# neoyinyao/Recommender

Measured on AMD Instinct MI355X. Metric: examples/sec fwd+bwd, Criteo-DLRM 26×40M×128 batch 65536, 1/2/4/8 GPU, higher is better.
Workload: dtype fp32; 1 GPU; dlrm_criteo_26x40000000x128; global_batch=65536, per_gpu_batch=65536, rows=40000000, dim=128, slots=26, optimizer=sgd, parallelism=single, prefetch=False

## Files before the change

### recommender_amd/csrc/interaction.hip

```cpp
#include <map>
#include <mutex>
#include <tuple>
#include <type_traits>

#include "common.hpp"

namespace rs {

int32_t fold_two_level(const float* part, int nchunks, int N, float* part2, float* out,
                       hipStream_t st);

typedef float floatx4 __attribute__((ext_vector_type(4)));
typedef float floatx16 __attribute__((ext_vector_type(16)));

struct InterMode {
  int self_interaction;
  int skip_gather;
};

__device__ __forceinline__ bool keep_pair(int i, int j, int self_i) {
  return self_i ? (i >= j) : (i < j);
}
__device__ __forceinline__ int compact_index(int i, int j, int F, int self_i) {
  return self_i ? (i * (i + 1) / 2 + j) : (i * F - i * (i + 1) / 2 + (j - i - 1));
// ... 434 lines not shown
      const float gsc = gscale[bb];
#pragma unroll
      for (int j = 0; j < GREG; ++j) gnx[j] = gsc * pv[j];
    } else {
      gfloat* grow = (gfloat*)(gout + bb * gstride);
#pragma unroll
      for (int j = 0; j < GREG; ++j) gnx[j] = grow[min(ln + 64 * j, glast)];
    }
  };
  const float* cur = row_of(first, raw_id(first));
  int64_t id_next = raw_id(first + 1);
#pragma unroll
  for (int s = 0; s < KS; ++s) load_rows(cur, s);
  load_g(first, lane);
  float* gs = gsm[wave];
  if (lane == 0) gs[ZS] = 0.f;
  for (int64_t b = first; b < last; ++b) {
    int lanev;
    asm volatile("v_mbcnt_lo_u32_b32 %0, -1, 0\n\tv_mbcnt_hi_u32_b32 %0, -1, %0" : "=v"(lanev));
    const int r = lanev & 31, h = lanev >> 5;
#pragma unroll
    for (int j = 0; j < GREG; ++j) gs[lane + 64 * j] = gnx[j];
    const float* nxt = row_of(b + 1, id_next);
    id_next = raw_id(b + 2);
    __builtin_amdgcn_s_waitcnt(0xc07f);
    __builtin_amdgcn_wave_barrier();
    float sa[KS];
#pragma unroll
    for (int s = 0; s < KS; ++s) {
      const int k = 2 * s + h;
      const bool in = r < F && k < F;
      const bool p1 = in && keep_pair(r, k, SELF);
      const bool p2 = in && keep_pair(k, r, SELF);
      const int j1 = p1 ? (SKIP ? r * F + k : compact_index(r, k, F, SELF)) : ZS;
      const int j2 = p2 ? (SKIP ? k * F + r : compact_index(k, r, F, SELF)) : ZS;
      sa[s] = gs[j1] + gs[j2];
    }
    floatx16 acc[NTILE];
#pragma unroll
    for (int c = 0; c < NTILE; ++c)
#pragma unroll
      for (int e = 0; e < 16; ++e) acc[c][e] = 0.f;
#pragma unroll
    for (int s = 0; s < KS; ++s) {
#pragma unroll
      for (int c = 0; c < NTILE; ++c)
        acc[c] = __builtin_amdgcn_mfma_f32_32x32x2f32(sa[s], xv[s][c], acc[c], 0, 0, 0);
    }
    __builtin_amdgcn_sched_barrier(0);
#pragma unroll
    for (int s = 0; s < KS; ++s) load_rows(nxt, s);
    __builtin_amdgcn_sched_barrier(0);
    float dpass[NTILE];
#pragma unroll
    for (int c = 0; c < NTILE; ++c) dpass[c] = gs[nz + NTILE * r + c];
    load_g(b + 1, lanev);
#pragma unroll
    for (int reg = 0; reg < 16; ++reg) {
      const int i = (reg & 3) + 8 * (reg >> 2) + 4 * h;
      if (i < F) {
        float v[NTILE];
#pragma unroll
        for (int c = 0; c < NTILE; ++c) v[c] = acc[c][reg] + (i == S ? dpass[c] : 0.f);
        float* dst = (i < S ? gemb + (b * S + i) * (int64_t)D : gdense + b * D) + NTILE * r;
        *reinterpret_cast<float4*>(dst) = make_float4(v[0], v[1], v[2], v[3]);
      }
    }
  }
  if (__any(oob) && lane == 0) flag_oob(src.err_flag);
}

constexpr int kDxLdx = 136;
constexpr int kDxRows = 28;
constexpr int kDxZt = 32 * 33;

template <bool ID64>
__global__ __launch_bounds__(256) void dlrm_fwd_dx_pipe(GatherSrc src, int64_t batch, int F,
                                                        float* __restrict__ out,
                                                        int64_t out_stride, FwdHead hd, int epw) {
  constexpr int D = 128, NT = 8;
  __shared__ __attribute__((aligned(16))) float lds[4][kDxRows * kDxLdx + kDxZt];
  const int wave = threadIdx.x >> 6, lane = threadIdx.x & 63;
  const int64_t first = ((int64_t)blockIdx.x * 4 + wave) * epw;
  if (first >= batch) return;
  const int64_t last = first + epw < batch ? first + epw : batch;
  const int r = lane & 15, g = lane >> 4;
  const int r32 = lane & 31, h = lane >> 5;
  const int S = src.n_slots;
  const int nzc = F * (F - 1) / 2;
  float* X = lds[wave];
  float(*z)[33] = reinterpret_cast<float(*)[33]>(lds[wave] + kDxRows * kDxLdx);
  float qz[8], qd[2], sa[2][8], qdn[4];
#pragma unroll
  for (int t = 0; t < 8; ++t) qz[t] = lane + 64 * t < nzc ? hd.q[lane + 64 * t] : 0.f;
#pragma unroll
  for (int t = 0; t < 2; ++t) qd[t] = hd.q[nzc + lane + 64 * t];
  const float cc = hd.c[0];
#pragma unroll
  for (int ib = 0; ib < 2; ++ib)
#pragma unroll
    for (int kk = 0; kk < 8; ++kk) {
      const int m = 16 * ib + r, k = 4 * kk + g;
      const bool in = m < F && k < F && m != k;
      const float v = hd.q[in ? compact_index(m < k ? m : k, m < k ? k : m, F, 0) : 0];
      sa[ib][kk] = in ? v : 0.f;
    }
#pragma unroll
  for (int c = 0; c < 4; ++c) qdn[c] = hd.q[nzc + 4 * r32 + c];
  int zoff[8];
#pragma unroll
  for (int t = 0; t < 8; ++t) {
    const int o = lane + 64 * t;
    int i = 0, j = 0;
    if (o < nzc) compact_pair(o, F, false, i, j);
    zoff[t] = o < nzc ? i * 33 + j : -1;
  }
  int64_t lo = 0, n_ok = src.n_rows;
  if (lane < S && src.slot_offsets) {
    lo = src.slot_offsets[lane];
    n_ok = src.slot_offsets[lane + 1] - lo;
  }
  bool oob = false;
  auto raw_id = [&](int64_t b) -> int64_t {
    const int64_t bb = b < last ? b : first;
    const int ln = lane < S ? lane : S - 1;
    const int64_t v = ID64 ? static_cast<const int64_t*>(src.ids)[bb * S + ln]
                           : static_cast<int64_t>(static_cast<const int32_t*>(src.ids)[bb * S + ln]);
    return lane < S ? v : 0;
  };
  auto row_of = [&](int64_t b, int64_t id) -> const float* {
    const bool live = b < last;
    const bool id_ok = id >= 0 && id < n_ok;
    if (lane < S && !id_ok && live) oob = true;
    if (lane < S) return id_ok ? src.table + (lo + id) * D : kZeroRow;
    return (lane == S && live) ? src.dense + (b < last ? b : first) * D : kZeroRow;
  };
  floatx4 a0[NT], a1[NT];
  float dnv[2];
  auto gather = [&](const float* mine, int64_t b) {
    const float* p0 = shfl_ptr(mine, r);
    const float* p1 = shfl_ptr(mine, 16 + r);
#pragma unroll
    for (int t = 0; t < NT; ++t) {
      a0[t] = *(gfloatx4*)(p0 + 4 * g + 16 * t);
      a1[t] = *(gfloatx4*)(p1 + 4 * g + 16 * t);
    }
    const int64_t bb = b < last ? b : first;
#pragma unroll
    for (int t = 0; t < 2; ++t) dnv[t] = *(gfloat*)(src.dense + bb * D + lane + 64 * t);
  };
  gather(row_of(first, raw_id(first)), first);
  int64_t id_next = raw_id(first + 1);
  for (int64_t b = first; b < last; ++b) {
    int lanev;
    asm volatile("v_mbcnt_lo_u32_b32 %0, -1, 0\n\tv_mbcnt_hi_u32_b32 %0, -1, %0" : "=v"(lanev));
    const int r = lanev & 15, g = (lanev >> 4) & 3;
    const int r32 = lanev & 31, h = (lanev >> 5) & 1;
    const float* nxt = row_of(b + 1, id_next);
    id_next = raw_id(b + 2);
    floatx4 c00 = {0.f, 0.f, 0.f, 0.f}, c01 = c00, c11 = c00;
#pragma unroll
    for (int t = 0; t < NT; ++t) {
#pragma unroll
      for (int c = 0; c < 4; ++c) {
        c00 = __builtin_amdgcn_mfma_f32_16x16x4f32(a0[t][c], a0[t][c], c00, 0, 0, 0);
        c01 = __builtin_amdgcn_mfma_f32_16x16x4f32(a0[t][c], a1[t][c], c01, 0, 0, 0);
        c11 = __builtin_amdgcn_mfma_f32_16x16x4f32(a1[t][c], a1[t][c], c11, 0, 0, 0);
      }
    }
#pragma unroll
    for (int t = 0; t < NT; ++t) {
      *reinterpret_cast<floatx4*>(&X[r * kDxLdx + 16 * t + 4 * g]) = a0[t];
      if (16 + r < kDxRows) *reinterpret_cast<floatx4*>(&X[(16 + r) * kDxLdx + 16 * t + 4 * g]) = a1[t];
    }
    float dn_cur[2] = {dnv[0], dnv[1]};
    __builtin_amdgcn_sched_barrier(0);
    gather(nxt, b + 1);
    __builtin_amdgcn_sched_barrier(0);
#pragma unroll
    for (int reg = 0; reg < 4; ++reg) {
      const int i = 4 * g + reg;
      z[i][r] = c00[reg];
      z[i][16 + r] = c01[reg];
      z[16 + r][i] = c01[reg];
      z[16 + i][16 + r] = c11[reg];
    }
    __builtin_amdgcn_wave_barrier();
    float* orow = out + b * out_stride;
    float hacc = 0.f;
    const int pad = nzc + D;
#pragma unroll
    for (int t = 0; t < 8; ++t) {
      const int o = lanev + 64 * t;
      const bool in = zoff[t] >= 0;
      const float v = in ? (&z[0][0])[zoff[t]] : 0.f;
      orow[in ? o : pad] = v;
      hacc += v * qz[t];
    }
    float* od = orow + nzc;
#pragma unroll
    for (int t = 0; t < 2; ++t) {
      const int d = lanev + 64 * t;
      od[d] = dn_cur[t];
      hacc += dn_cur[t] * qd[t];
    }
#pragma unroll
    for (int off = 32; off > 0; off >>= 1) hacc += __shfl_xor(hacc, off);
    {
      const float v = hacc + cc;
      hd.y[b] = hd.act == 2 ? 1.f / (1.f + expf(-v)) : (hd.act == 1 ? fmaxf(v, 0.f) : v);
    }
    {
      const int o = pad + lanev;
      orow[o < out_stride ? o : pad] = 0.f;
    }
#pragma unroll
    for (int t = 0; t < NT; ++t) {
      constexpr int KK = kDxRows / 4;
      float bv[KK];
#pragma unroll
      for (int kk = 0; kk < KK; ++kk) bv[kk] = X[(4 * kk + g) * kDxLdx + 16 * t + r];
      floatx4 d0 = {0.f, 0.f, 0.f, 0.f}, d1 = d0;
#pragma unroll
      for (int kk = 0; kk < KK; ++kk) {
        d0 = __builtin_amdgcn_mfma_f32_16x16x4f32(sa[0][kk], bv[kk], d0, 0, 0, 0);
        d1 = __builtin_amdgcn_mfma_f32_16x16x4f32(sa[1][kk], bv[kk], d1, 0, 0, 0);
      }
#pragma unroll
      for (int reg = 0; reg < 4; ++reg) {
        const int i0 = 4 * g + reg, i1 = 16 + 4 * g + reg;
        X[i0 * kDxLdx + 16 * t + r] = d0[reg];
        if (i1 < kDxRows) X[i1 * kDxLdx + 16 * t + r] = d1[reg];
      }
    }
    __builtin_amdgcn_wave_barrier();
    float* de = hd.dxu_emb + b * S * (int64_t)D;
#pragma unroll
    for (int s2 = 0; s2 < kDxRows / 2; ++s2) {
      const int i = 2 * s2 + h < S ? 2 * s2 + h : S;
      floatx4 v = *reinterpret_cast<const floatx4*>(&X[i * kDxLdx + 4 * r32]);
      const bool emb = i < S;
#pragma unroll
      for (int c = 0; c < 4; ++c) v[c] = emb ? v[c] : v[c] + qdn[c];
      float* dst = emb ? de + i * D : hd.dxu_dense + b * D;
      *reinterpret_cast<floatx4*>(dst + 4 * r32) = v;
    }
    __builtin_amdgcn_wave_barrier();
  }
  if (__any(oob) && lane == 0) flag_oob(src.err_flag);
}

typedef __bf16 bf16x8 __attribute__((ext_vector_type(8)));

typedef __bf16 bf16x2 __attribute__((ext_vector_type(2)));
typedef float floatx2 __attribute__((ext_vector_type(2)));
__device__ __forceinline__ void split3(const floatx4& lo, const floatx4& hi, bf16x8& h, bf16x8& m,
                                       bf16x8& l) {
#pragma unroll
  for (int j = 0; j < 4; ++j) {
    const floatx2 x = j < 2 ? floatx2{lo[2 * j], lo[2 * j + 1]} : floatx2{hi[2 * j - 4], hi[2 * j - 3]};
    const bf16x2 hp = __builtin_convertvector(x, bf16x2);
    const floatx2 r1 = x - __builtin_convertvector(hp, floatx2);
    const bf16x2 mp = __builtin_convertvector(r1, bf16x2);
    const bf16x2 lp = __builtin_convertvector(r1 - __builtin_convertvector(mp, floatx2), bf16x2);
    h[2 * j] = hp[0];
    h[2 * j + 1] = hp[1];
    m[2 * j] = mp[0];
    m[2 * j + 1] = mp[1];
    l[2 * j] = lp[0];
    l[2 * j + 1] = lp[1];
  }
}

__device__ __forceinline__ floatx4 mfma6(const bf16x8& ah, const bf16x8& am, const bf16x8& al,
                                         const bf16x8& bh, const bf16x8& bm, const bf16x8& bl,
                                         floatx4 c) {
  c = __builtin_amdgcn_mfma_f32_16x16x32_bf16(am, bm, c, 0, 0, 0);
  c = __builtin_amdgcn_mfma_f32_16x16x32_bf16(ah, bl, c, 0, 0, 0);
  c = __builtin_amdgcn_mfma_f32_16x16x32_bf16(al, bh, c, 0, 0, 0);
  c = __builtin_amdgcn_mfma_f32_16x16x32_bf16(ah, bm, c, 0, 0, 0);
  c = __builtin_amdgcn_mfma_f32_16x16x32_bf16(am, bh, c, 0, 0, 0);
  return __builtin_amdgcn_mfma_f32_16x16x32_bf16(ah, bh, c, 0, 0, 0);
}

constexpr int kTrainAtop = 512;
constexpr int kTrainNI = 13;
template <int D>
constexpr int train_m() { return kTrainAtop + 2 + kTrainNI * D + D; }
constexpr int kTrainM = train_m<128>();

struct TrainArgs {
  const float* q;
  const float* c;
  const float* label;
  const float* xin;
  float eps;
  float gscale;
  float* y;
  float* grad_emb;
  float* part;
};

typedef short shortx4 __attribute__((ext_vector_type(4)));
typedef short shortx8 __attribute__((ext_vector_type(8)));
typedef __attribute__((address_space(3))) shortx4 lds_shortx4;

__device__ __forceinline__ floatx4 mfma6_xs(const bf16x8& xh, const bf16x8& xm, const bf16x8& xl,
                                            const bf16x8& sh, const bf16x8& sm, const bf16x8& sl,
                                            floatx4 c) {
  c = __builtin_amdgcn_mfma_f32_16x16x32_bf16(xm, sm, c, 0, 0, 0);
  c = __builtin_amdgcn_mfma_f32_16x16x32_bf16(xl, sh, c, 0, 0, 0);
  c = __builtin_amdgcn_mfma_f32_16x16x32_bf16(xh, sl, c, 0, 0, 0);
  c = __builtin_amdgcn_mfma_f32_16x16x32_bf16(xm, sh, c, 0, 0, 0);
  c = __builtin_amdgcn_mfma_f32_16x16x32_bf16(xh, sm, c, 0, 0, 0);
  return __builtin_amdgcn_mfma_f32_16x16x32_bf16(xh, sh, c, 0, 0, 0);
}

constexpr int kChPlane = 32 * 32 * 2;
constexpr int kChImage = 3 * kChPlane;
__device__ __forceinline__ int ch_off(int row, int col) {
  const int chunk = (col >> 3) ^ ((row >> 1) & 3) ^ (((row >> 3) & 1) << 1);
  return row * 64 + 16 * chunk + 2 * (col & 7);
}
constexpr int kChStageLd = 36;
template <int D>
constexpr int chunk_region_floats() {
  return (kChImage / 4 + 32 * kChStageLd + D) > train_m<D>() ? (kChImage / 4 + 32 * kChStageLd + D)
                                                             : train_m<D>();
}

template <int D, bool ID64>
__global__ __launch_bounds__(256, 2) void dlrm_train_chunk(GatherSrc src, int64_t batch, int F,
                                                        TrainArgs ta, float* g_rows, int epw) {
  static_assert(D == 64 || D == 128, "train kernel laid out for D = 64 or 128");
  constexpr int NT = D / 16, NC = D / 32, DL = D / 4, RPI = 64 / DL, DPL = D / 64;
  constexpr int TM = train_m<D>();
  constexpr int RW = chunk_region_floats<D>();
  __shared__ __attribute__((aligned(16))) float lds[4][RW];
  __shared__ __attribute__((aligned(16))) float qlane[64][12];
  __shared__ __attribute__((aligned(16))) float qsh[kTrainAtop];
  __shared__ __attribute__((aligned(16))) bf16x8 sash[2][3][64];
  const int wave = threadIdx.x >> 6, lane = threadIdx.x & 63;
  const int64_t first = ((int64_t)blockIdx.x * 4 + wave) * epw;
  const int64_t last = first + epw < batch ? first + epw : batch;
  const bool active = first < batch;
  const int r = lane & 15, g = lane >> 4;
  const int S = src.n_slots;
  const int nzc = F * (F - 1) / 2;
  char* img = reinterpret_cast<char*>(lds[wave]);
  float* stg = lds[wave] + kChImage / 4;
  float* ubot = stg + 32 * kChStageLd;
  for (int e = threadIdx.x; e < kTrainAtop; e += 256) {
    const float v = ta.q[e < nzc + D ? e : 0];
    qsh[e] = e < nzc + D ? v : 0.f;
  }
  if (wave == 0) {
    float qv[12];
    bool qk[12];
#pragma unroll
    for (int reg = 0; reg < 4; ++reg) {
      const int i0 = 4 * g + reg, j0 = r;
      const int i1 = 4 * g + reg, j1 = 16 + r;
      const int i2 = 16 + 4 * g + reg, j2 = 16 + r;
      qk[reg] = i0 < j0 && j0 < F;
      qk[4 + reg] = j1 < F;
      qk[8 + reg] = i2 < j2 && j2 < F;
      qv[reg] = ta.q[qk[reg] ? compact_index(i0, j0, F, 0) : 0];
      qv[4 + reg] = ta.q[qk[4 + reg] ? compact_index(i1, j1, F, 0) : 0];
      qv[8 + reg] = ta.q[qk[8 + reg] ? compact_index(i2, j2, F, 0) : 0];
    }
#pragma unroll
    for (int k = 0; k < 12; ++k) qlane[lane][k] = qk[k] ? qv[k] : 0.f;
  }
  if (wave == 1) {
#pragma unroll
    for (int ib = 0; ib < 2; ++ib) {
      floatx4 v[2];
#pragma unroll
      for (int j = 0; j < 8; ++j) {
        const int m = 16 * ib + r, kk = 8 * g + j;
        const bool in = m < F && kk < F && m != kk;
        const float q = ta.q[in ? compact_index(m < kk ? m : kk, m < kk ? kk : m, F, 0) : 0];
        v[j >> 2][j & 3] = in ? q : 0.f;
      }
      split3(v[0], v[1], sash[ib][0][lane], sash[ib][1][lane], sash[ib][2][lane]);
    }
  }
  __syncthreads();
  const float cc = ta.c[0];
  float az[12], ad[4], abot[DPL][kTrainNI], sbot[DPL];
  float s_top = 0.f, loss = 0.f;
#pragma unroll
  for (int k = 0; k < 12; ++k) az[k] = 0.f;
#pragma unroll
  for (int k = 0; k < 4; ++k) ad[k] = 0.f;
#pragma unroll
  for (int k = 0; k < DPL; ++k) {
    sbot[k] = 0.f;
#pragma unroll
    for (int i = 0; i < kTrainNI; ++i) abot[k][i] = 0.f;
  }
  int64_t lo = 0, n_ok = src.n_rows;
  if (lane < S && src.slot_offsets) {
    lo = src.slot_offsets[lane];
    n_ok = src.slot_offsets[lane + 1] - lo;
  }
  bool oob = false;
  auto raw_id = [&](int64_t b) -> int64_t {
    const int64_t bb = b < last ? b : first;
    const int ln = lane < S ? lane : S - 1;
    const int64_t v = ID64 ? static_cast<const int64_t*>(src.ids)[bb * S + ln]
                           : static_cast<int64_t>(static_cast<const int32_t*>(src.ids)[bb * S + ln]);
    return lane < S ? v : 0;
  };
  auto row_of = [&](int64_t b, int64_t id) -> const float* {
    const bool live = b < last;
    const bool id_ok = id >= 0 && id < n_ok;
    if (lane < S && !id_ok && live) oob = true;
    if (lane < S) return id_ok ? src.table + (lo + id) * D : kZeroRow;
    return (lane == S && live) ? src.dense + (b < last ? b : first) * D : kZeroRow;
  };
  floatx4 a0[NT], a1[NT];
  floatx4 dn4;
  const float* p0 = nullptr;
  const float* p1 = nullptr;
  auto load_chunk = [&](int s) {
    a0[2 * s] = *(gfloatx4*)(p0 + 32 * s + 8 * g);
    a0[2 * s + 1] = *(gfloatx4*)(p0 + 32 * s + 8 * g + 4);
    a1[2 * s] = *(gfloatx4*)(p1 + 32 * s + 8 * g);
    a1[2 * s + 1] = *(gfloatx4*)(p1 + 32 * s + 8 * g + 4);
  };
  auto load_side = [&](int64_t b) {
    const int cl = lane & (DL - 1);
    const int64_t bb = b < last ? b : first;
    dn4 = *(gfloatx4*)(src.dense + bb * D + 4 * cl);
  };
  if (active) {
    {
      const float* mine = row_of(first, raw_id(first));
      p0 = shfl_ptr(mine, r);
      p1 = shfl_ptr(mine, 16 + r);
      load_side(first);
#pragma unroll
      for (int s = 0; s < NC; ++s) load_chunk(s);
    }
    int64_t id_next = raw_id(first + 1);
    for (int64_t b = first; b < last; ++b) {
      int lanev;
      asm volatile("v_mbcnt_lo_u32_b32 %0, -1, 0\n\tv_mbcnt_hi_u32_b32 %0, -1, %0" : "=v"(lanev));
      const int r = lanev & 15, g = (lanev >> 4) & 3;
      {
        const float* nxt = row_of(b + 1, id_next);
        p0 = shfl_ptr(nxt, r);
        p1 = shfl_ptr(nxt, 16 + r);
      }
      id_next = raw_id(b + 2);
      const floatx4 dn = dn4;
      float xb[kTrainNI];
      typedef __attribute__((address_space(4))) const float cfloat;
      const int bq = __builtin_amdgcn_readfirstlane((int)b);
      const cfloat* xr = (const cfloat*)(ta.xin + (int64_t)bq * kTrainNI);
#pragma unroll
      for (int i = 0; i < kTrainNI; ++i) xb[i] = xr[i];
      const float lb = ((const cfloat*)ta.label)[bq];
      load_side(b + 1);
      float* de = ta.grad_emb + b * S * (int64_t)D;
      floatx4 c00 = {0.f, 0.f, 0.f, 0.f}, c01 = c00, c11 = c00;
      const int q = (lanev >> 2) & 3, p4 = lanev & 3;
#pragma unroll
      for (int s = 0; s < NC; ++s) {
        bf16x8 sa[2][3];
#pragma unroll
        for (int ib = 0; ib < 2; ++ib)
#pragma unroll
          for (int pt = 0; pt < 3; ++pt) sa[ib][pt] = sash[ib][pt][lanev & 63];
        bf16x8 h0, m0, l0, h1, m1, l1;
        split3(a0[2 * s], a0[2 * s + 1], h0, m0, l0);
        split3(a1[2 * s], a1[2 * s + 1], h1, m1, l1);
        __builtin_amdgcn_sched_barrier(0);
        load_chunk(s);
        __builtin_amdgcn_sched_barrier(0);
        c00 = mfma6(h0, m0, l0, h0, m0, l0, c00);
        c01 = mfma6(h0, m0, l0, h1, m1, l1, c01);
        c11 = mfma6(h1, m1, l1, h1, m1, l1, c11);
        *reinterpret_cast<bf16x8*>(img + 0 * kChPlane + ch_off(r, 8 * g)) = h0;
        *reinterpret_cast<bf16x8*>(img + 1 * kChPlane + ch_off(r, 8 * g)) = m0;
        *reinterpret_cast<bf16x8*>(img + 2 * kChPlane + ch_off(r, 8 * g)) = l0;
        *reinterpret_cast<bf16x8*>(img + 0 * kChPlane + ch_off(16 + r, 8 * g)) = h1;
        *reinterpret_cast<bf16x8*>(img + 1 * kChPlane + ch_off(16 + r, 8 * g)) = m1;
        *reinterpret_cast<bf16x8*>(img + 2 * kChPlane + ch_off(16 + r, 8 * g)) = l1;
        __builtin_amdgcn_wave_barrier();
#pragma unroll
        for (int tt = 0; tt < 2; ++tt) {
          bf16x8 xp[3];
#pragma unroll
          for (int pt = 0; pt < 3; ++pt) {
            const int o0 = pt * kChPlane + ch_off(8 * g + q, 16 * tt + 4 * p4);
            const int o1 = pt * kChPlane + ch_off(8 * g + 4 + q, 16 * tt + 4 * p4);
            const shortx4 lo4 =
                __builtin_amdgcn_ds_read_tr16_b64_v4i16((lds_shortx4*)(img + o0));
            const shortx4 hi4 =
                __builtin_amdgcn_ds_read_tr16_b64_v4i16((lds_shortx4*)(img + o1));
            const shortx8 v8 = __builtin_shufflevector(lo4, hi4, 0, 1, 2, 3, 4, 5, 6, 7);
            xp[pt] = __builtin_bit_cast(bf16x8, v8);
          }
          floatx4 d0 = {0.f, 0.f, 0.f, 0.f}, d1 = d0;
          d0 = mfma6_xs(xp[0], xp[1], xp[2], sa[0][0], sa[0][1], sa[0][2], d0);
          d1 = mfma6_xs(xp[0], xp[1], xp[2], sa[1][0], sa[1][1], sa[1][2], d1);
          const int col = 16 * tt + 4 * g;
          *reinterpret_cast<floatx4*>(stg + r * kChStageLd + col) = d0;
          *reinterpret_cast<floatx4*>(stg + (16 + r) * kChStageLd + col) = d1;
          if (r == S) *reinterpret_cast<floatx4*>(ubot + 32 * s + col) = d0;
          if (16 + r == S) *reinterpret_cast<floatx4*>(ubot + 32 * s + col) = d1;
        }
        __builtin_amdgcn_wave_barrier();
#pragma unroll
        for (int pp = 0; pp < 4; ++pp) {
          const int i = 8 * pp + (lanev >> 3), c8 = lanev & 7;
          const floatx4 v = *reinterpret_cast<const floatx4*>(stg + i * kChStageLd + 4 * c8);
          if (i < S)
            __builtin_nontemporal_store(v, reinterpret_cast<floatx4*>(de + i * D + 32 * s + 4 * c8));
        }
        __builtin_amdgcn_wave_barrier();
      }
      const int cl = lanev & (DL - 1), rg = (lanev / DL) & (RPI - 1);
      float zr[12];
#pragma unroll
      for (int reg = 0; reg < 4; ++reg) {
        zr[reg] = c00[reg];
        zr[4 + reg] = c01[reg];
        zr[8 + reg] = c11[reg];
      }
      float hacc = 0.f;
      {
        const floatx4* ql = reinterpret_cast<const floatx4*>(&qlane[lanev & 63][0]);
#pragma unroll
        for (int q4 = 0; q4 < 3; ++q4) {
          const floatx4 qv = ql[q4];
#pragma unroll
          for (int k = 0; k < 4; ++k) hacc += zr[4 * q4 + k] * qv[k];
        }
        const floatx4 qd = *reinterpret_cast<const floatx4*>(&qsh[nzc + 4 * cl]);
        if (rg == 0) {
#pragma unroll
          for (int k = 0; k < 4; ++k) hacc += dn[k] * qd[k];
        }
      }
#pragma unroll
      for (int off = 32; off > 0; off >>= 1) hacc += __shfl_xor(hacc, off);
      const float p = 1.f / (1.f + expf(-(hacc + cc)));
      {
        const float pc = fminf(fmaxf(p, ta.eps), 1.f - ta.eps);
        loss += -(lb * logf(pc + ta.eps) + (1.f - lb) * logf((1.f - pc) + ta.eps));
      }
      const bool inside = p >= ta.eps && p <= 1.f - ta.eps;
      const float pcg = fminf(fmaxf(p, ta.eps), 1.f - ta.eps);
      const float dbce = -(lb / (pcg + ta.eps)) + (1.f - lb) / ((1.f - pcg) + ta.eps);
      const float dp = inside ? ta.gscale * dbce : 0.f;
      const float G = dp * (p * (1.f - p));
      if (lanev == 0) {
        ta.y[b] = p;
        g_rows[b] = G;
      }
      s_top += G;
#pragma unroll
      for (int k = 0; k < 12; ++k) az[k] += zr[k] * G;
#pragma unroll
      for (int k = 0; k < 4; ++k) ad[k] += dn[k] * G;
      {
        const floatx4 v = *reinterpret_cast<const floatx4*>(ubot + 4 * cl);
        const floatx4 qdn = *reinterpret_cast<const floatx4*>(&qsh[nzc + 4 * cl]);
#pragma unroll
        for (int k = 0; k < DPL; ++k) {
          const int c = DPL * rg + k;
          const float gd = __fmul_rn(G, v[c] + qdn[c]);
          const float gb = dn[c] > 0.f ? gd : 0.f;
          sbot[k] += gb;
#pragma unroll
          for (int ii = 0; ii < kTrainNI; ++ii) abot[k][ii] += xb[ii] * gb;
        }
      }
      __builtin_amdgcn_wave_barrier();
    }
  }
  __syncthreads();
  float* X = lds[wave];
  for (int e = lane; e < TM; e += 64) X[e] = 0.f;
  __builtin_amdgcn_wave_barrier();
  if (active) {
    const int cl = lane & (DL - 1), rg = lane / DL;
#pragma unroll
    for (int reg = 0; reg < 4; ++reg) {
      const int i0 = 4 * g + reg, j0 = r, i1 = 4 * g + reg, j1 = 16 + r, i2 = 16 + 4 * g + reg, j2 = 16 + r;
      if (i0 < j0 && j0 < F) X[compact_index(i0, j0, F, 0)] = az[reg];
      if (j1 < F) X[compact_index(i1, j1, F, 0)] = az[4 + reg];
      if (i2 < j2 && j2 < F) X[compact_index(i2, j2, F, 0)] = az[8 + reg];
    }
    if (rg == 0) {
#pragma unroll
      for (int k = 0; k < 4; ++k) X[nzc + 4 * cl + k] = ad[k];
    }
    if (lane == 0) {
      X[kTrainAtop] = s_top;
      X[kTrainAtop + 1] = loss;
    }
#pragma unroll
    for (int k = 0; k < DPL; ++k) {
      const int d = 4 * cl + DPL * rg + k;
#pragma unroll
      for (int ii = 0; ii < kTrainNI; ++ii) X[kTrainAtop + 2 + ii * D + d] = abot[k][ii];
      X[kTrainAtop + 2 + kTrainNI * D + d] = sbot[k];
    }
  }
  __syncthreads();
  for (int e = threadIdx.x; e < TM; e += 256) {
    float v = lds[0][e];
    v += lds[1][e];
    v += lds[2][e];
    v += lds[3][e];
    ta.part[(int64_t)blockIdx.x * TM + e] = v;
  }
  if (__any(oob) && lane == 0) flag_oob(src.err_flag);
}


template <int GREG, int KS, bool ID64>
static void launch_pipe_t(const GatherSrc& src, int64_t batch, int F, InterMode md,
                          const float* gout, int64_t gstride, float* gemb, float* gdense, int,
                          hipStream_t st, const float* gscale = nullptr) {
  auto go = [&](auto kern) {
    const int epw = pipe_epw(reinterpret_cast<const void*>(kern), batch);
    kern<<<ceil_div(batch, 4 * (int64_t)epw), 256, 0, st>>>(src, batch, F, gout, gstride, gemb,
                                                           gdense, epw, gscale);
  };
  if (gscale) {
    go(dlrm_bwd_pipe<128, GREG, KS, false, false, ID64, true>);
    return;
  }
  if (md.self_interaction) {
    if (md.skip_gather) go(dlrm_bwd_pipe<128, GREG, KS, true, true, ID64>);
    else go(dlrm_bwd_pipe<128, GREG, KS, true, false, ID64>);
  } else {
    if (md.skip_gather) go(dlrm_bwd_pipe<128, GREG, KS, false, true, ID64>);
    else go(dlrm_bwd_pipe<128, GREG, KS, false, false, ID64>);
  }
}

template <int GREG, int KS>
static void launch_pipe(const GatherSrc& src, int64_t batch, int F, InterMode md,
                        const float* gout, int64_t gstride, float* gemb, float* gdense, int epw,
                        hipStream_t st, const float* gscale = nullptr) {
  if (src.id_dtype == RS_ID_I64)
    launch_pipe_t<GREG, KS, true>(src, batch, F, md, gout, gstride, gemb, gdense, epw, st, gscale);
  else
    launch_pipe_t<GREG, KS, false>(src, batch, F, md, gout, gstride, gemb, gdense, epw, st, gscale);
}

template <class Src, bool DLRM_OUT>
__global__ __launch_bounds__(64) void inter_fwd_generic(Src src, int64_t batch, int F, int D,
                                                        InterMode md, float* __restrict__ out,
                                                        int64_t out_stride) {
  extern __shared__ __attribute__((aligned(16))) float xs[];
  const int lane = threadIdx.x;
  const int64_t b = blockIdx.x;
  const int ld = D + 1;
  bool oob = false;
  for (int i = 0; i < F; ++i) {
    const float* xr = src.row(b, i, D, oob);
    for (int d = lane; d < D; d += 64) xs[i * ld + d] = xr ? xr[d] : 0.f;
  }
  __syncthreads();
  float* orow = out + b * out_stride;
  for (int o = lane; o < F * F; o += 64) {
    int i = o / F, j = o - i * F;
    bool keep = keep_pair(i, j, md.self_interaction);
    if (!keep && !md.skip_gather) continue;
    float s = 0.f;
    if (keep)
      for (int d = 0; d < D; ++d) s = fmaf(xs[i * ld + d], xs[j * ld + d], s);
    if (md.skip_gather)
      orow[o] = s;
    else
      orow[compact_index(i, j, F, md.self_interaction)] = s;
  }
  if constexpr (DLRM_OUT) {
    const int nz = out_width(F, md.self_interaction, md.skip_gather);
    float* od = orow + nz;
    for (int d = lane; d < D; d += 64) od[d] = src.dense[b * D + d];
    for (int64_t o = nz + D + lane; o < out_stride; o += 64) orow[o] = 0.f;
    if (__any(oob) && lane == 0) flag_oob(src.err_flag);
  }
}

template <class Src, bool DLRM_OUT>
__global__ __launch_bounds__(64) void inter_bwd_generic(Src src, int64_t batch, int F, int D,
                                                        InterMode md, const float* __restrict__ gout,
                                                        int64_t gstride, float* __restrict__ gx,
                                                        float* __restrict__ gemb,
                                                        float* __restrict__ gdense) {
  extern __shared__ __attribute__((aligned(16))) float sm[];
  float* xs = sm;
  float* ss = sm + F * (D + 1);
  const int lane = threadIdx.x;
  const int64_t b = blockIdx.x;
  const int ld = D + 1, ls = F + 1;
  bool oob = false;
  const float* grow = gout + b * gstride;
  for (int i = 0; i < F; ++i) {
    const float* xr = src.row(b, i, D, oob);
    for (int d = lane; d < D; d += 64) xs[i * ld + d] = xr ? xr[d] : 0.f;
  }
  for (int o = lane; o < F * F; o += 64) {
    int i = o / F, k = o - i * F;
    float v = 0.f;
    if (keep_pair(i, k, md.self_interaction))
      v += md.skip_gather ? grow[i * F + k] : grow[compact_index(i, k, F, md.self_interaction)];
    if (keep_pair(k, i, md.self_interaction))
      v += md.skip_gather ? grow[k * F + i] : grow[compact_index(k, i, F, md.self_interaction)];
    ss[i * ls + k] = v;
  }
  __syncthreads();
  for (int o = lane; o < F * D; o += 64) {
    int i = o / D, d = o - i * D;
    float s = 0.f;
    for (int k = 0; k < F; ++k) s = fmaf(ss[i * ls + k], xs[k * ld + d], s);
    if constexpr (DLRM_OUT) {
      if (i < src.n_slots) {
        gemb[(b * src.n_slots + i) * (int64_t)D + d] = s;
      } else {
        gdense[b * D + d] = s + grow[out_width(F, md.self_interaction, md.skip_gather) + d];
      }
    } else {
      gx[(b * F + i) * (int64_t)D + d] = s;
    }
  }
}

__global__ __launch_bounds__(256) void fm_fwd_kernel(const float* __restrict__ emb, int64_t batch,
                                                     int F, int D, float* __restrict__ out) {
  const int wave = threadIdx.x >> 6, lane = threadIdx.x & 63;
  const int64_t b = (int64_t)blockIdx.x * 4 + wave;
  if (b >= batch) return;
  const float* e = emb + b * F * (int64_t)D;
  float part = 0.f;
  for (int d = lane; d < D; d += 64) {
    float s = 0.f, q = 0.f;
    for (int f = 0; f < F; ++f) {
      float x = e[f * D + d];
      s += x;
      q += x * x;
    }
    part += s * s - q;
  }
  for (int off = 32; off > 0; off >>= 1) part += __shfl_down(part, off);
  if (lane == 0) out[b] = 0.5f * part;
}

__global__ __launch_bounds__(256) void fm_bwd_kernel(const float* __restrict__ emb,
                                                     const float* __restrict__ gout, int64_t batch,
                                                     int F, int D, float* __restrict__ gemb) {
  const int wave = threadIdx.x >> 6, lane = threadIdx.x & 63;
  const int64_t b = (int64_t)blockIdx.x * 4 + wave;
  if (b >= batch) return;
  const float* e = emb + b * F * (int64_t)D;
  float* ge = gemb + b * F * (int64_t)D;
  const float g = gout[b];
  for (int d = lane; d < D; d += 64) {
    float s = 0.f;
    for (int f = 0; f < F; ++f) s += e[f * D + d];
    for (int f = 0; f < F; ++f) ge[f * D + d] = g * (s - e[f * D + d]);
  }
}

template <class Src, bool DLRM_OUT>
static int32_t launch_fwd(const Src& src, int64_t batch, int F, int D, InterMode md, float* out,
                          int64_t out_stride, bool aligned16, hipStream_t st) {
  if (batch == 0) return RS_OK;
  if (F <= 32 && aligned16) {
    int64_t blocks = ceil_div(batch, 4);
    switch (D) {
      case 16: inter_fwd_mfma<16, Src, DLRM_OUT><<<blocks, 256, 0, st>>>(src, batch, F, md, out, out_stride); RS_CHECK_LAUNCH(); return RS_OK;
      case 32: inter_fwd_mfma<32, Src, DLRM_OUT><<<blocks, 256, 0, st>>>(src, batch, F, md, out, out_stride); RS_CHECK_LAUNCH(); return RS_OK;
      case 64: inter_fwd_mfma<64, Src, DLRM_OUT><<<blocks, 256, 0, st>>>(src, batch, F, md, out, out_stride); RS_CHECK_LAUNCH(); return RS_OK;
      case 128: inter_fwd_mfma<128, Src, DLRM_OUT><<<blocks, 256, 0, st>>>(src, batch, F, md, out, out_stride); RS_CHECK_LAUNCH(); return RS_OK;
      case 256: inter_fwd_mfma<256, Src, DLRM_OUT><<<blocks, 256, 0, st>>>(src, batch, F, md, out, out_stride); RS_CHECK_LAUNCH(); return RS_OK;
      default: break;
    }
  }
  size_t lds = (size_t)F * (D + 1) * 4;
  if (lds > 64 * 1024) {
    set_error("interaction F=%d D=%d too large for the generic kernel", F, D);
    return RS_E_UNSUPPORTED;
  }
  inter_fwd_generic<Src, DLRM_OUT><<<batch, 64, lds, st>>>(src, batch, F, D, md, out, out_stride);
  RS_CHECK_LAUNCH();
  return RS_OK;
}

template <class Src, bool DLRM_OUT>
static int32_t launch_bwd(const Src& src, int64_t batch, int F, int D, InterMode md,
                          const float* gout, int64_t gstride, float* gx, float* gemb, float* gdense,
                          bool aligned16, hipStream_t st) {
  if (batch == 0) return RS_OK;
  if constexpr (DLRM_OUT && std::is_same<Src, GatherSrc>::value) {
    const int epw = kPipeEPW;
    const int gw = out_width(F, md.self_interaction, md.skip_gather) + D;
    if (F <= 32 && aligned16 && D == 128 && gw <= 20 * 64) {
      const bool k14 = F <= 28;
      if (gw <= 8 * 64) {
        if (k14) launch_pipe<8, 14>(src, batch, F, md, gout, gstride, gemb, gdense, epw, st);
        else launch_pipe<8, 16>(src, batch, F, md, gout, gstride, gemb, gdense, epw, st);
        RS_CHECK_LAUNCH();
        return RS_OK;
      }
      {
        if (k14) launch_pipe<20, 14>(src, batch, F, md, gout, gstride, gemb, gdense, epw, st);
        else launch_pipe<20, 16>(src, batch, F, md, gout, gstride, gemb, gdense, epw, st);
        RS_CHECK_LAUNCH();
        return RS_OK;
      }
    }
  }
  if (F <= 32 && aligned16) {
    int64_t blocks = ceil_div(batch, 4);
    switch (D) {
      case 32: inter_bwd_mfma<32, Src, DLRM_OUT><<<blocks, 256, 0, st>>>(src, batch, F, md, gout, gstride, gx, gemb, gdense); RS_CHECK_LAUNCH(); return RS_OK;
      case 64: inter_bwd_mfma<64, Src, DLRM_OUT><<<blocks, 256, 0, st>>>(src, batch, F, md, gout, gstride, gx, gemb, gdense); RS_CHECK_LAUNCH(); return RS_OK;
      case 128: inter_bwd_mfma<128, Src, DLRM_OUT><<<blocks, 256, 0, st>>>(src, batch, F, md, gout, gstride, gx, gemb, gdense); RS_CHECK_LAUNCH(); return RS_OK;
      default: break;
    }
  }
  size_t lds = ((size_t)F * (D + 1) + (size_t)F * (F + 1)) * 4;
  if (lds > 64 * 1024) {
    set_error("interaction F=%d D=%d too large for the generic kernel", F, D);
    return RS_E_UNSUPPORTED;
  }
  inter_bwd_generic<Src, DLRM_OUT><<<batch, 64, lds, st>>>(src, batch, F, D, md, gout, gstride, gx,
                                                           gemb, gdense);
  RS_CHECK_LAUNCH();
  return RS_OK;
}

static bool al16(const void* p) { return (reinterpret_cast<uintptr_t>(p) & 15) == 0; }

}

using namespace rs;

extern "C" int32_t rs_dot_interaction_fwd(const float* x, int64_t batch, int32_t F, int32_t D,
                                          int32_t self_interaction, int32_t skip_gather, float* out,
                                          int64_t out_stride, void* stream) {
  RS_CHECK_ARG(F >= 1 && D >= 1 && batch >= 0, "bad sizes");
  RS_CHECK_ARG(out_stride >= out_width(F, self_interaction, skip_gather), "out_stride too small");
  RS_CHECK_ARG(batch == 0 || (x && out), "null pointer");
  DenseSrc src{x, F};
  return launch_fwd<DenseSrc, false>(src, batch, F, D, {self_interaction, skip_gather}, out,
                                     out_stride, al16(x), as_stream(stream));
}

extern "C" int32_t rs_dot_interaction_bwd(const float* x, const float* grad_out, int64_t batch,
                                          int32_t F, int32_t D, int32_t self_interaction,
                                          int32_t skip_gather, int64_t grad_stride, float* grad_x,
                                          void* stream) {
  RS_CHECK_ARG(F >= 1 && D >= 1 && batch >= 0, "bad sizes");
  RS_CHECK_ARG(grad_stride >= out_width(F, self_interaction, skip_gather), "grad_stride too small");
  RS_CHECK_ARG(batch == 0 || (x && grad_out && grad_x), "null pointer");
  DenseSrc src{x, F};
  return launch_bwd<DenseSrc, false>(src, batch, F, D, {self_interaction, skip_gather}, grad_out,
                                     grad_stride, grad_x, nullptr, nullptr, al16(x) && al16(grad_x),
                                     as_stream(stream));
}

extern "C" int32_t rs_dlrm_interaction_fwd(const float* table, int64_t n_rows, int32_t D,
                                           const void* ids, int32_t id_dtype, int32_t n_slots,
                                           const int64_t* slot_offsets, const float* dense,
                                           int64_t batch, int32_t compact, float* out,
                                           int64_t out_stride, int32_t* err_flag, void* stream) {
  const int F = n_slots + 1;
  const InterMode md{0, compact ? 0 : 1};
  RS_CHECK_ARG(n_slots >= 1 && D >= 1 && batch >= 0, "bad sizes");
  RS_CHECK_ARG(id_dtype == RS_ID_I32 || id_dtype == RS_ID_I64, "bad id dtype");
  RS_CHECK_ARG(out_stride >= out_width(F, 0, md.skip_gather) + D, "out_stride too small");
  RS_CHECK_ARG(batch == 0 || (table && ids && dense && out), "null pointer");
  GatherSrc src{table, n_rows, ids, id_dtype, n_slots, slot_offsets, dense, err_flag};
  return launch_fwd<GatherSrc, true>(src, batch, F, D, md, out, out_stride,
// ... 229 lines not shown
```

Baseline: 107.5 million examples/sec.

## Use buffer stores for grad_emb and outputs; keep bottom-grad row in registers

Replaces the guarded nontemporal global stores of per-sample embedding gradients with raw buffer stores whose range clamps out-of-slot rows, so the i<S branch goes away. The extra ubot LDS row is dropped: each lane pulls its slice of row S from the staging tile into registers. Scalar y/G writes become range-limited buffer stores, the dense dot is computed branch-free, and a per-sample wave barrier is removed. The goal is fewer branches, less LDS traffic and sync per sample, and better store scheduling, at the cost of relying on buffer out-of-range semantics for correctness.

```diff
diff --git a/recommender_amd/csrc/interaction.hip b/recommender_amd/csrc/interaction.hip
--- a/recommender_amd/csrc/interaction.hip
+++ b/recommender_amd/csrc/interaction.hip
@@ -760,6 +760,7 @@
 };
 
 typedef short shortx4 __attribute__((ext_vector_type(4)));
+typedef unsigned uintx4 __attribute__((ext_vector_type(4)));
 typedef short shortx8 __attribute__((ext_vector_type(8)));
 typedef __attribute__((address_space(3))) shortx4 lds_shortx4;
 
@@ -783,8 +784,8 @@
 constexpr int kChStageLd = 36;
 template <int D>
 constexpr int chunk_region_floats() {
-  return (kChImage / 4 + 32 * kChStageLd + D) > train_m<D>() ? (kChImage / 4 + 32 * kChStageLd + D)
-                                                             : train_m<D>();
+  return (kChImage / 4 + 32 * kChStageLd) > train_m<D>() ? (kChImage / 4 + 32 * kChStageLd)
+                                                         : train_m<D>();
 }
 
 template <int D, bool ID64>
@@ -807,7 +808,6 @@
   const int nzc = F * (F - 1) / 2;
   char* img = reinterpret_cast<char*>(lds[wave]);
   float* stg = lds[wave] + kChImage / 4;
-  float* ubot = stg + 32 * kChStageLd;
   for (int e = threadIdx.x; e < kTrainAtop; e += 256) {
     const float v = ta.q[e < nzc + D ? e : 0];
     qsh[e] = e < nzc + D ? v : 0.f;
@@ -922,7 +922,9 @@
       for (int i = 0; i < kTrainNI; ++i) xb[i] = xr[i];
       const float lb = ((const cfloat*)ta.label)[bq];
       load_side(b + 1);
-      float* de = ta.grad_emb + b * S * (int64_t)D;
+      const __amdgpu_buffer_rsrc_t de_rs = __builtin_amdgcn_make_buffer_rsrc(
+          ta.grad_emb + (int64_t)bq * S * D, 0, S * D * 4, 0x00020000);
+      floatx4 ub = {0.f, 0.f, 0.f, 0.f};
       floatx4 c00 = {0.f, 0.f, 0.f, 0.f}, c01 = c00, c11 = c00;
       const int q = (lanev >> 2) & 3, p4 = lanev & 3;
 #pragma unroll
@@ -968,16 +970,28 @@
           const int col = 16 * tt + 4 * g;
           *reinterpret_cast<floatx4*>(stg + r * kChStageLd + col) = d0;
           *reinterpret_cast<floatx4*>(stg + (16 + r) * kChStageLd + col) = d1;
-          if (r == S) *reinterpret_cast<floatx4*>(ubot + 32 * s + col) = d0;
-          if (16 + r == S) *reinterpret_cast<floatx4*>(ubot + 32 * s + col) = d1;
         }
         __builtin_amdgcn_wave_barrier();
-#pragma unroll
-        for (int pp = 0; pp < 4; ++pp) {
-          const int i = 8 * pp + (lanev >> 3), c8 = lanev & 7;
-          const floatx4 v = *reinterpret_cast<const floatx4*>(stg + i * kChStageLd + 4 * c8);
-          if (i < S)
-            __builtin_nontemporal_store(v, reinterpret_cast<floatx4*>(de + i * D + 32 * s + 4 * c8));
+        {
+          const int c8 = lanev & 7;
+          floatx4 rv[4];
+#pragma unroll
+          for (int pp = 0; pp < 4; ++pp) {
+            const int i = 8 * pp + (lanev >> 3);
+            rv[pp] = *reinterpret_cast<const floatx4*>(stg + i * kChStageLd + 4 * c8);
+          }
+          const floatx4 v = *reinterpret_cast<const floatx4*>(stg + S * kChStageLd + 4 * c8);
+          __builtin_amdgcn_sched_group_barrier(0x100, 5, 0);
+          __builtin_amdgcn_sched_group_barrier(0x040, 4, 0);
+#pragma unroll
+          for (int pp = 0; pp < 4; ++pp) {
+            const int i = 8 * pp + (lanev >> 3);
+            __builtin_amdgcn_raw_buffer_store_b128(__builtin_bit_cast(uintx4, rv[pp]), de_rs,
+                                                   (i * D + 32 * s + 4 * c8) * 4, 0, 2);
+          }
+          const bool mine = ((lanev & (DL - 1)) >> 3) == s;
+#pragma unroll
+          for (int k = 0; k < 4; ++k) ub[k] = mine ? v[k] : ub[k];
         }
         __builtin_amdgcn_wave_barrier();
       }
@@ -999,10 +1013,10 @@
           for (int k = 0; k < 4; ++k) hacc += zr[4 * q4 + k] * qv[k];
         }
         const floatx4 qd = *reinterpret_cast<const floatx4*>(&qsh[nzc + 4 * cl]);
-        if (rg == 0) {
-#pragma unroll
-          for (int k = 0; k < 4; ++k) hacc += dn[k] * qd[k];
-        }
+        float hd = hacc;
+#pragma unroll
+        for (int k = 0; k < 4; ++k) hd += dn[k] * qd[k];
+        hacc = rg == 0 ? hd : hacc;
       }
 #pragma unroll
       for (int off = 32; off > 0; off >>= 1) hacc += __shfl_xor(hacc, off);
@@ -1016,17 +1030,19 @@
       const float dbce = -(lb / (pcg + ta.eps)) + (1.f - lb) / ((1.f - pcg) + ta.eps);
       const float dp = inside ? ta.gscale * dbce : 0.f;
       const float G = dp * (p * (1.f - p));
-      if (lanev == 0) {
-        ta.y[b] = p;
-        g_rows[b] = G;
-      }
+      __builtin_amdgcn_raw_buffer_store_b32(
+          __float_as_uint(p), __builtin_amdgcn_make_buffer_rsrc(ta.y + bq, 0, 4, 0x00020000),
+          4 * (lanev & 63), 0, 0);
+      __builtin_amdgcn_raw_buffer_store_b32(
+          __float_as_uint(G), __builtin_amdgcn_make_buffer_rsrc(g_rows + bq, 0, 4, 0x00020000),
+          4 * (lanev & 63), 0, 0);
       s_top += G;
 #pragma unroll
       for (int k = 0; k < 12; ++k) az[k] += zr[k] * G;
 #pragma unroll
       for (int k = 0; k < 4; ++k) ad[k] += dn[k] * G;
       {
-        const floatx4 v = *reinterpret_cast<const floatx4*>(ubot + 4 * cl);
+        const floatx4 v = ub;
         const floatx4 qdn = *reinterpret_cast<const floatx4*>(&qsh[nzc + 4 * cl]);
 #pragma unroll
         for (int k = 0; k < DPL; ++k) {
@@ -1038,7 +1054,6 @@
           for (int ii = 0; ii < kTrainNI; ++ii) abot[k][ii] += xb[ii] * gb;
         }
       }
-      __builtin_amdgcn_wave_barrier();
     }
   }
   __syncthreads();
```

Measured after the change: 107.1 million examples/sec. About the same (-0.4%).
